# ylsung/vl-merging

Hardware: NVIDIA B200
Metric: gram_cache_samples_per_sec (higher is better)
Workload: dtype tf32

## Files before the change

### include/vlmerge.h

```cpp
#ifndef VLMERGE_H_
#define VLMERGE_H_

#include <stddef.h>
#include <stdint.h>

#ifdef __cplusplus
extern "C" {
#endif

#define VLM_ABI_VERSION 3

typedef enum {
  VLM_OK = 0,
  VLM_ERR_INVALID_ARG = -1,
  VLM_ERR_ALIGNMENT = -2,
  VLM_ERR_UNSUPPORTED = -3,
  VLM_ERR_DRIVER = -4,
  VLM_ERR_NOT_SPD = -5,
  VLM_ERR_INTERNAL = -6
} vlm_status;

typedef enum {
  VLM_F32 = 0, VLM_BF16 = 1, VLM_F16 = 2, VLM_F64 = 3,
  VLM_TF32X2 = 4
} vlm_dtype;

int         vlm_version(void);
const char* vlm_last_error(void);
uint64_t    vlm_launch_count(void);

int vlm_syrk_accum(const void* x, int dtype, int64_t rows, int d, int64_t ldx,
                   float* g, int64_t ldg, void* stream);

int vlm_tf32_split(const float* x, int64_t rows, int d, int64_t ldx, int64_t seg_rows, int64_t seg_stride,
                   float* out, void* stream);

int vlm_syrk_accum_f64(const void* x, int dtype, int64_t rows, int d, int64_t ldx, int64_t seg_rows,
                       int64_t seg_stride, double* g, int64_t ldg, void* stream);

uint64_t vlm_syrk_i8x4_scratch_bytes(int64_t rows, int d);
int vlm_syrk_accum_i8x4(const void* x, int dtype, int64_t rows, int d, int64_t ldx, int64_t seg_rows, int64_t seg_stride,
                        void* scratch, uint64_t scratch_bytes, double* g, int64_t ldg, void* stream);

typedef struct {
  const void* x;
  int64_t     rows;
  int64_t     ldx;
  float*      g;
  int64_t     ldg;
  int32_t     d;
  int32_t     reserved;
  int64_t     seg_rows;
  int64_t     seg_stride;
} vlm_syrk_problem;
int vlm_syrk_accum_batch(const vlm_syrk_problem* probs_host, int n, int dtype, void* stream);

int vlm_syrk_accum_strided(const void* x, int dtype, int64_t rows, int d, int64_t ldx, int64_t seg_rows,
                           int64_t seg_stride, float* g, int64_t ldg, void* stream);

int vlm_syrk_accum_simt(const void* x, int dtype, int64_t rows, int d, int64_t ldx,
                        float* g, int64_t ldg, void* stream);

typedef struct vlm_sym_item {
  const void* full;
  void* packed;
  int32_t d;
  int32_t reserved;
  int64_t ld;
} vlm_sym_item;
int vlm_sym_pack_upper_batch(const vlm_sym_item* items, int n, int dtype, void* stream);
int vlm_sym_unpack_batch(const vlm_sym_item* items, int n, int dtype, void* stream);
int vlm_sym_mirror_batch(const vlm_sym_item* items, int n, int dtype, void* stream);

typedef struct vlm_sym_span {
  uint64_t offset_bytes;
  int32_t d;
  int32_t reserved;
  int64_t ld;
} vlm_sym_span;
int vlm_sym_allreduce_multimem(void* multicast_base, const vlm_sym_span* spans, int n, int dtype, int rank, int world,
                               void* stream);

int vlm_syrk_pair_schedule_host(int64_t rows, int d, int elem_bytes, int nsm, int32_t* segs_out, int cap,
                                int32_t* off_out, int off_cap, int* ncluster_out);

typedef enum { VLM_MERGE_WSUM = 0, VLM_MERGE_SEQ_LERP = 1, VLM_MERGE_MEAN = 2 } vlm_merge_mode;
#define VLM_MERGE_MAX_SRC 4

typedef struct {
  float*       dst;
  const float* src[VLM_MERGE_MAX_SRC];
  float        coef[VLM_MERGE_MAX_SRC];
  uint64_t     n;
  int32_t      n_src;
  int32_t      mode;
} vlm_merge_seg;

typedef struct vlm_merge_plan vlm_merge_plan;
int vlm_merge_plan_create(const vlm_merge_seg* segs_host, int n_seg, vlm_merge_plan** out);
int vlm_merge_plan_run(const vlm_merge_plan* plan, void* stream);
int vlm_merge_plan_destroy(vlm_merge_plan* plan);
uint64_t vlm_merge_plan_bytes(const vlm_merge_plan* plan);

int vlm_copy_batch(void* dst_base, const uint64_t* dst_off_bytes, const void* const* src_host_or_dev,
                   const uint64_t* nbytes, int n, void* stream);

int vlm_gram_scale_accum(const void* g, int g_dtype, int d, int64_t ldg, double alpha,
                         double* out, int64_t ldo, int accumulate, void* stream);
int vlm_regmean_rhs(const float* w, int out_f, int in_f, int64_t ldw,
                    const void* g, int g_dtype, int64_t ldg, double alpha,
                    double* acc, int64_t ldacc, int accumulate, void* stream);
int vlm_regmean_rhs_diff(const float* w, const float* w_base, int out_f, int in_f, int64_t ldw,
                         const void* g, int g_dtype, int64_t ldg, double alpha,
                         double* acc, int64_t ldacc, int accumulate, void* stream);
int vlm_widen_add(const float* src, int rows, int cols, int64_t lds, double* dst, int64_t ldd, void* stream);
int vlm_spd_solve_right(double* s, int in_f, int64_t lds, double* r, int out_f, int64_t ldr,
                        void* stream);
int vlm_spd_solve_right_async(double* s, int in_f, int64_t lds, double* r, int out_f, int64_t ldr,
                              int* info_dev, void* stream);

int vlm_sim_topk_splits(int64_t m, int64_t n);
int vlm_sim_topk(const void* a, int64_t m, int64_t lda, const void* b, int64_t n, int64_t ldb, int d, int dtype,
                 float* out_val, int32_t* out_idx, int splits, void* stream);

int vlm_lu_solve_right(double* s, int in_f, int64_t lds, double* r, int out_f, int64_t ldr, void* stream);

#ifdef __cplusplus
}
#endif
#endif
```

### vl-merging_b200/_lib.py

```python
import ctypes
import itertools
import os
import subprocess
from ctypes import POINTER, c_char_p, c_double, c_float, c_int, c_int32, c_int64, c_uint64, c_void_p

_PKG_DIR = os.path.dirname(os.path.abspath(__file__))
LIB_PATH = os.path.join(_PKG_DIR, "libvlmerge.so")
CSRC_DIR = os.path.join(_PKG_DIR, "csrc")

VLM_F32, VLM_BF16, VLM_F16, VLM_F64, VLM_TF32X2 = 0, 1, 2, 3, 4
MERGE_WSUM, MERGE_SEQ_LERP, MERGE_MEAN = 0, 1, 2
MERGE_MAX_SRC = 4
ERR_NOT_SPD = -5


class MergeSeg(ctypes.Structure):
    _fields_ = [
        ("dst", c_void_p),
        ("src", c_void_p * MERGE_MAX_SRC),
        ("coef", c_float * MERGE_MAX_SRC),
        ("n", c_uint64),
        ("n_src", c_int32),
        ("mode", c_int32),
    ]


class SymItem(ctypes.Structure):
    _fields_ = [("full", c_void_p), ("packed", c_void_p), ("d", c_int32), ("reserved", c_int32), ("ld", c_int64)]


def sym_items(grams, packed=None, offsets=None):
    items = (SymItem * len(grams))()
    if offsets is None:
        offsets = itertools.accumulate((g.shape[0] * (g.shape[0] + 1) // 2 for g in grams), initial=0)
    for it, g, off in zip(items, grams, offsets):
        it.full, it.d, it.ld = g.data_ptr(), g.shape[0], g.stride(0)
        if packed is not None:
            it.packed = packed.data_ptr() + packed.element_size() * off
    return items


class SymSpan(ctypes.Structure):
    _fields_ = [("offset_bytes", ctypes.c_uint64), ("d", c_int32), ("reserved", c_int32), ("ld", c_int64)]


class SyrkProblem(ctypes.Structure):
    _fields_ = [
        ("x", c_void_p),
        ("rows", c_int64),
        ("ldx", c_int64),
        ("g", c_void_p),
        ("ldg", c_int64),
        ("d", c_int32),
        ("reserved", c_int32),
        ("seg_rows", c_int64),
        ("seg_stride", c_int64),
    ]


class VlmError(RuntimeError):
    def __init__(self, code, msg):
        super().__init__(f"libvlmerge error {code}: {msg}")
        self.code = code


SIGNATURES = {
    "vlm_version": (c_int, []),
    "vlm_last_error": (c_char_p, []),
    "vlm_launch_count": (c_uint64, []),
    "vlm_syrk_accum": (c_int, [c_void_p, c_int, c_int64, c_int, c_int64, c_void_p, c_int64, c_void_p]),
    "vlm_tf32_split": (c_int, [c_void_p, c_int64, c_int, c_int64, c_int64, c_int64, c_void_p, c_void_p]),
    "vlm_syrk_accum_f64": (c_int, [c_void_p, c_int, c_int64, c_int, c_int64, c_int64, c_int64, c_void_p, c_int64,
                                   c_void_p]),
    "vlm_syrk_i8x4_scratch_bytes": (c_uint64, [c_int64, c_int]),
    "vlm_syrk_accum_i8x4": (c_int, [c_void_p, c_int, c_int64, c_int, c_int64, c_int64, c_int64, c_void_p, c_uint64,
                                    c_void_p, c_int64, c_void_p]),
    "vlm_syrk_accum_batch": (c_int, [POINTER(SyrkProblem), c_int, c_int, c_void_p]),
    "vlm_syrk_accum_strided": (c_int, [c_void_p, c_int, c_int64, c_int, c_int64, c_int64, c_int64, c_void_p, c_int64,
                                       c_void_p]),
    "vlm_syrk_accum_simt": (c_int, [c_void_p, c_int, c_int64, c_int, c_int64, c_void_p, c_int64, c_void_p]),
    "vlm_sym_pack_upper_batch": (c_int, [POINTER(SymItem), c_int, c_int, c_void_p]),
    "vlm_sym_unpack_batch": (c_int, [POINTER(SymItem), c_int, c_int, c_void_p]),
    "vlm_sym_allreduce_multimem": (c_int, [c_void_p, POINTER(SymSpan), c_int, c_int, c_int, c_int, c_void_p]),
    "vlm_sym_mirror_batch": (c_int, [POINTER(SymItem), c_int, c_int, c_void_p]),
    "vlm_syrk_pair_schedule_host": (c_int, [c_int64, c_int, c_int, c_int, POINTER(c_int32), c_int, POINTER(c_int32),
                                            c_int, POINTER(c_int)]),
    "vlm_merge_plan_create": (c_int, [POINTER(MergeSeg), c_int, POINTER(c_void_p)]),
    "vlm_merge_plan_run": (c_int, [c_void_p, c_void_p]),
    "vlm_merge_plan_destroy": (c_int, [c_void_p]),
    "vlm_merge_plan_bytes": (c_uint64, [c_void_p]),
    "vlm_copy_batch": (c_int, [c_void_p, POINTER(c_uint64), POINTER(c_void_p), POINTER(c_uint64), c_int, c_void_p]),
    "vlm_gram_scale_accum": (c_int, [c_void_p, c_int, c_int, c_int64, c_double, c_void_p, c_int64, c_int, c_void_p]),
    "vlm_regmean_rhs": (c_int, [c_void_p, c_int, c_int, c_int64, c_void_p, c_int, c_int64, c_double, c_void_p,
                                c_int64, c_int, c_void_p]),
    "vlm_regmean_rhs_diff": (c_int, [c_void_p, c_void_p, c_int, c_int, c_int64, c_void_p, c_int, c_int64, c_double,
                                     c_void_p, c_int64, c_int, c_void_p]),
    "vlm_widen_add": (c_int, [c_void_p, c_int, c_int, c_int64, c_void_p, c_int64, c_void_p]),
    "vlm_spd_solve_right": (c_int, [c_void_p, c_int, c_int64, c_void_p, c_int, c_int64, c_void_p]),
    "vlm_sim_topk_splits": (c_int, [c_int64, c_int64]),
    "vlm_sim_topk": (c_int, [c_void_p, c_int64, c_int64, c_void_p, c_int64, c_int64, c_int, c_int, c_void_p, c_void_p, c_int,
                             c_void_p]),
    "vlm_lu_solve_right": (c_int, [c_void_p, c_int, c_int64, c_void_p, c_int, c_int64, c_void_p]),
    "vlm_spd_solve_right_async": (c_int, [c_void_p, c_int, c_int64, c_void_p, c_int, c_int64, c_void_p, c_void_p]),
}

_lib = None


def build(verbose=False):
    res = subprocess.run(["make", "-C", CSRC_DIR, f"-j{min(8, os.cpu_count() or 1)}", "all"], capture_output=True, text=True)
    if verbose or res.returncode != 0:
        print(res.stdout[-4000:])
        print(res.stderr[-4000:])
    if res.returncode != 0:
        raise RuntimeError("building libvlmerge.so failed (see output above)")
    return LIB_PATH


def lib():
    global _lib
    if _lib is None:
        if not os.path.exists(LIB_PATH):
            raise RuntimeError(
                f"{LIB_PATH} not found: build it with `python -c 'import __graft_entry__ as g; g.build()'` "
                "or `make -C vl-merging_b200/csrc`.  There is no CPU fallback for the merge hot path.")
        h = ctypes.CDLL(LIB_PATH)
        for name, (restype, argtypes) in SIGNATURES.items():
            fn = getattr(h, name)
            fn.restype = restype
            fn.argtypes = argtypes
        if h.vlm_version() != 3:
            raise RuntimeError(f"libvlmerge ABI version {h.vlm_version()} != 3: rebuild it (make -C vl-merging_b200/csrc)")
        _lib = h
    return _lib


def check(rc):
    if rc != 0:
        raise VlmError(rc, lib().vlm_last_error().decode(errors="replace"))


def launch_count():
    return int(lib().vlm_launch_count())


def syrk_pair_schedule(rows, d, elem_bytes=4, nsm=148):
    cap = 1 << 16
    segs = (c_int32 * (4 * cap))()
    off = (c_int32 * (nsm + 2))()
    ncl = c_int(0)
    n = lib().vlm_syrk_pair_schedule_host(rows, d, elem_bytes, nsm, segs, cap, off, nsm + 2, ctypes.byref(ncl))
    if n < 0:
        check(n)
    return [tuple(segs[4 * i: 4 * i + 4]) for i in range(n)], list(off[: ncl.value + 1])
```

### vl-merging_b200/model.py

```python
import math

import torch
import torch.nn as nn
import torch.nn.functional as F

MODALITIES = ("v", "l", "vl")


class Mlp(nn.Module):
    def __init__(self, dim, hidden):
        super().__init__()
        self.fc1 = nn.Linear(dim, hidden)
        self.act = nn.GELU()
        self.fc2 = nn.Linear(hidden, dim)

    def forward(self, x):
        return self.fc2(self.act(self.fc1(x)))


class Attention(nn.Module):

    def __init__(self, dim, num_heads, attn_impl="reference"):
        super().__init__()
        self.num_heads = num_heads
        self.scale = (dim // num_heads) ** -0.5
        self.attn_impl = attn_impl
        self.qkv = nn.Linear(dim, dim * 3, bias=False)
        self.q_bias = nn.Parameter(torch.zeros(dim))
        self.v_bias = nn.Parameter(torch.zeros(dim))
        self.proj = nn.Linear(dim, dim)

    def forward(self, x, mask=None, relative_position_bias=None):
        b, n, c = x.shape
        bias = torch.cat((self.q_bias, torch.zeros_like(self.v_bias), self.v_bias))
        qkv = F.linear(x, self.qkv.weight, bias).reshape(b, n, 3, self.num_heads, -1).permute(2, 0, 3, 1, 4)
        if self.attn_impl == "sdpa":
            add = relative_position_bias.unsqueeze(0).to(qkv.dtype) if relative_position_bias is not None else None
            if mask is not None and not bool(mask.all()):
                pad = torch.zeros(b, 1, 1, n, dtype=qkv.dtype, device=x.device).masked_fill(
                    ~mask.bool()[:, None, None, :], float("-inf"))
                add = pad if add is None else add + pad
            x = F.scaled_dot_product_attention(qkv[0], qkv[1], qkv[2], attn_mask=add, scale=self.scale)
            return self.proj(x.transpose(1, 2).reshape(b, n, c))
        q, k, v = qkv[0] * self.scale, qkv[1], qkv[2]
        attn = q.float() @ k.float().transpose(-2, -1)
        if relative_position_bias is not None:
            attn = attn + relative_position_bias.unsqueeze(0)
        if mask is not None:
            attn = attn.masked_fill(~mask.bool()[:, None, None, :], float("-inf"))
        attn = attn.softmax(dim=-1).type_as(x)
        x = (attn @ v).transpose(1, 2).reshape(b, n, c)
        return self.proj(x)


class Block(nn.Module):

    def __init__(self, dim, num_heads, mlp_ratio, experts, attn_impl="reference", joint=False, max_text_len=40):
        super().__init__()
        self.experts = experts
        self.joint = joint
        self.max_text_len = max_text_len
        hidden = int(dim * mlp_ratio)
        ln = lambda: nn.LayerNorm(dim, eps=1e-6)
        if experts is None:
            self.attn, self.norm1 = Attention(dim, num_heads, attn_impl), ln()
            self.mlp, self.norm2 = Mlp(dim, hidden), ln()
        else:
            self.attn = nn.ModuleDict({m: Attention(dim, num_heads, attn_impl) for m in experts})
            self.norm1 = nn.ModuleDict({m: ln() for m in experts})
            self.mlp = nn.ModuleDict({m: Mlp(dim, hidden) for m in experts})
            self.norm2 = nn.ModuleDict({m: ln() for m in experts})
        self.gamma_1 = nn.Parameter(0.1 * torch.ones(dim))
        self.gamma_2 = nn.Parameter(0.1 * torch.ones(dim))

    def forward(self, x, mask, type_id, relative_position_bias):
        if type_id == 2 and not self.joint:
            return self._forward_split(x, mask, relative_position_bias)
        if self.experts is None:
            attn, norm1, mlp, norm2 = self.attn, self.norm1, self.mlp, self.norm2
        else:
            m = MODALITIES[type_id]
            attn, norm1, mlp, norm2 = self.attn[m], self.norm1[m], self.mlp[m], self.norm2[m]
        x = x + self.gamma_1 * attn(norm1(x), mask=mask, relative_position_bias=relative_position_bias)
        x = x + self.gamma_2 * mlp(norm2(x))
        return x

    def _forward_split(self, x, mask, bias):
        L = self.max_text_len
        moe = self.experts is not None
        pick = (lambda mod, m: mod[m]) if moe else (lambda mod, m: mod)
        h = torch.cat([pick(self.norm1, "l")(x[:, :L]), pick(self.norm1, "v")(x[:, L:])], dim=1)
        a_t = pick(self.attn, "l")(h[:, :L], mask=mask[:, :L], relative_position_bias=bias[:, :L, :L])
        a_i = pick(self.attn, "v")(h[:, L:], mask=mask[:, L:], relative_position_bias=bias[:, L:, L:])
        x = x + self.gamma_1 * torch.cat([a_t, a_i], dim=1)
        h = torch.cat([pick(self.norm2, "l")(x[:, :L]), pick(self.norm2, "v")(x[:, L:])], dim=1)
        x = x + self.gamma_2 * torch.cat([pick(self.mlp, "l")(h[:, :L]), pick(self.mlp, "v")(h[:, L:])], dim=1)
        return x


class PatchEmbed(nn.Module):
    def __init__(self, patch_size, dim):
        super().__init__()
        self.proj = nn.Conv2d(3, dim, kernel_size=patch_size, stride=patch_size)

    def forward(self, x):
        return self.proj(x)


class Transformer(nn.Module):
    def __init__(self, cfg, experts_for_layer):
        super().__init__()
        dim = cfg["hidden_size"]
        self.patch_embed = PatchEmbed(cfg["patch_size"], dim)
        self.cls_token = nn.Parameter(torch.zeros(1, 1, dim))
        self.mask_token = nn.Parameter(torch.zeros(1, 1, dim))
        self.blocks = nn.ModuleList(
            [Block(dim, cfg["num_heads"], cfg["mlp_ratio"], experts_for_layer(i), cfg.get("attn_impl", "reference"),
                   joint=i >= cfg["vlffn_start_layer_index"], max_text_len=cfg["max_text_len"])
             for i in range(cfg["num_layers"])])
        self.norm = nn.LayerNorm(dim, eps=1e-6)

    def visual_embed(self, img):
        x = self.patch_embed(img).flatten(2).transpose(1, 2)
        x = torch.cat((self.cls_token.expand(x.shape[0], -1, -1), x), dim=1)
        return x, torch.ones(x.shape[0], x.shape[1], device=x.device)


class TextEmbeddings(nn.Module):

    def __init__(self, vocab_size, dim, max_len):
        super().__init__()
        self.word_embeddings = nn.Embedding(vocab_size, dim, padding_idx=0)
        self.position_embeddings = nn.Embedding(max_len, dim)
        self.token_type_embeddings = nn.Embedding(2, dim)
        self.LayerNorm = nn.LayerNorm(dim, eps=1e-12)

    def forward(self, ids):
        pos = torch.arange(ids.shape[1], device=ids.device)
        x = self.word_embeddings(ids) + self.token_type_embeddings(torch.zeros_like(ids))
        return self.LayerNorm(x + self.position_embeddings(pos)[None])


class _Head(nn.Module):
    def __init__(self, dim, bias):
        super().__init__()
        setattr(self, "fc" if not bias else "dense", nn.Linear(dim, dim, bias=bias))


DEFAULT_CONFIG = dict(
    hidden_size=768, num_heads=12, num_layers=12, mlp_ratio=4, image_size=384, patch_size=16,
    max_text_len=40, max_text_len_of_initckpt=196, vocab_size=30522, vlffn_start_layer_index=10,
    use_moe=True, attn_impl="reference",
)


def vlmo_config(name="base", **overrides):
    cfg = dict(DEFAULT_CONFIG)
    if name == "large":
        cfg.update(hidden_size=1024, num_heads=16, num_layers=24, vlffn_start_layer_index=21)
    elif name == "tiny":
        cfg.update(hidden_size=192, num_heads=3, image_size=224)
    elif name != "base":
        raise ValueError(name)
    cfg.update(overrides)
    return cfg


class VLMo(nn.Module):

    def __init__(self, cfg):
        super().__init__()
        self.cfg = dict(cfg)
        dim, heads, layers = cfg["hidden_size"], cfg["num_heads"], cfg["num_layers"]
        self.num_layers = layers
        self.text_embeddings = TextEmbeddings(cfg["vocab_size"], dim, cfg["max_text_len"])
        self.token_type_embeddings = nn.Embedding(2, dim)
        vl0 = cfg["vlffn_start_layer_index"]
        if cfg["use_moe"]:
            experts = lambda i: ("v", "l") if i < vl0 else ("v", "l", "vl")
        else:
            experts = lambda i: None
        self.transformer = Transformer(cfg, experts)
        self.pooler = _Head(dim, bias=True)
        self.ifm_text_proj = _Head(dim, bias=False)
        self.ifm_image_proj = _Head(dim, bias=False)
        self.logit_scale = nn.Parameter(torch.ones([]) * math.log(1 / 0.07))

        w = cfg["image_size"] // cfg["patch_size"]
        max_text, init_text = cfg["max_text_len"], cfg["max_text_len_of_initckpt"]
        n_img = (2 * w - 1) * (2 * w - 1) + 3
        n_all = n_img + 2 * init_text + 2
        self.relative_position_bias_table = nn.Parameter(torch.zeros(n_all, heads * layers))
        ys, xs = torch.meshgrid(torch.arange(w), torch.arange(w), indexing="ij")
        coords = torch.stack((ys.flatten(), xs.flatten()))
        rel = (coords[:, :, None] - coords[:, None, :]).permute(1, 2, 0)
        idx = torch.zeros(w * w + 1, w * w + 1, dtype=torch.long)
        idx[1:, 1:] = (rel[..., 0] + w - 1) * (2 * w - 1) + rel[..., 1] + w - 1
        idx[0, :] = n_img - 3
        idx[:, 0] = n_img - 2
        idx[0, 0] = n_img - 1
        self.register_buffer("relative_position_index", idx)
        pos = torch.arange(max_text - 1)
        tidx = torch.zeros(max_text, max_text, dtype=torch.long)
        tidx[1:, 1:] = (pos[None, :] - pos[:, None]) - (2 - init_text) + n_img + 2
        tidx[0, :] = n_all - 3
        tidx[:, 0] = n_all - 2
        tidx[0, 0] = n_all - 1
        self.register_buffer("text_relative_position_index", tidx)
        t2i = torch.full((max_text, w * w + 1), float(n_img))
        i2t = torch.full((w * w + 1, max_text), float(n_img + 1))
        self.register_buffer("text_imag_relative_position_index",
                             torch.cat((torch.cat((tidx.float(), t2i), 1), torch.cat((i2t, idx.float()), 1)), 0))

    def _rel_pos_bias(self, index):
        bias = F.embedding(index, self.relative_position_bias_table).permute(2, 0, 1).contiguous()
        return torch.chunk(bias, self.num_layers, dim=0)

    def infer_text_ft(self, batch):
        ids, masks = batch["text_ids"], batch["text_masks"]
        x = self.text_embeddings(ids) + self.token_type_embeddings(torch.zeros_like(masks))
        biases = self._rel_pos_bias(self.text_relative_position_index)
        for i, blk in enumerate(self.transformer.blocks):
            x = blk(x, masks, 1, biases[i])
        feats = self.transformer.norm(x)
        cls = self.ifm_text_proj.fc(feats[:, 0])
        return {"text_feats": feats, "cls_feats": cls / cls.norm(dim=-1, keepdim=True), "raw_cls_feats": x[:, 0]}

    def infer_image_ft(self, batch, image_token_type_idx=1):
        img = batch["image"][0] if isinstance(batch["image"], (list, tuple)) else batch["image"]
        x, masks = self.transformer.visual_embed(img)
        masks = masks.long()
        x = x + self.token_type_embeddings(torch.full_like(masks, image_token_type_idx))
        biases = self._rel_pos_bias(self.relative_position_index)
        for i, blk in enumerate(self.transformer.blocks):
            x = blk(x, masks, 0, biases[i])
        feats = self.transformer.norm(x)
        cls = self.ifm_image_proj.fc(feats[:, 0])
        return {"image_feats": feats, "cls_feats": cls / cls.norm(dim=-1, keepdim=True), "raw_cls_feats": x[:, 0]}

    def infer(self, batch, image_token_type_idx=1):
        img = batch["image"][0] if isinstance(batch["image"], (list, tuple)) else batch["image"]
        ids, text_masks = batch["text_ids"], batch["text_masks"]
        text = self.text_embeddings(ids)
        image, image_masks = self.transformer.visual_embed(img)
        image_masks = image_masks.type_as(text_masks)
        text = text + self.token_type_embeddings(torch.zeros_like(text_masks))
        image = image + self.token_type_embeddings(torch.full_like(image_masks, image_token_type_idx))
        x = torch.cat([text, image], dim=1)
        masks = torch.cat([text_masks, image_masks], dim=1)
        biases = self._rel_pos_bias(self.text_imag_relative_position_index.long())
        for i, blk in enumerate(self.transformer.blocks):
            x = blk(x, masks, 2, biases[i])
        x = self.transformer.norm(x)
        n_text = text.shape[1]
        return {"text_feats": x[:, :n_text], "image_feats": x[:, n_text:],
                "cls_feats": torch.tanh(self.pooler.dense(x[:, 0])), "raw_cls_feats": x[:, 0]}

    def forward(self, batch):
        img = self.infer_image_ft(batch)["cls_feats"]
        txt = self.infer_text_ft(batch)["cls_feats"]
        return self.logit_scale.exp() * img @ txt.t()



def _hash_uniform(numel, seed, device="cpu"):
    i = torch.arange(numel, dtype=torch.int64, device=device)
    x = ((i + 1) * 0x9E3779B1 + (seed % (1 << 24)) * 0x85EBCA77 + 0x165667B1) % (1 << 32)
    x = (x ^ (x >> 15)) * 0x2C1B3C6D % (1 << 32)
    x = (x ^ (x >> 12)) * 0x297A2D39 % (1 << 32)
    x = x ^ (x >> 15)
    return ((x % (1 << 24)).to(torch.float32) + 0.5) / float(1 << 24) - 0.5


@torch.no_grad()
def init_synthetic_(model, seed=1):
    import zlib

    for name, p in model.named_parameters():
        u = _hash_uniform(p.numel(), seed * 1000003 + zlib.crc32(name.encode()) % 999983, device=p.device).reshape(p.shape)
        if "norm" in name.lower() and name.endswith("weight"):
            p.copy_(1.0 + 0.2 * u)
        elif "gamma_" in name:
            p.copy_(0.1 + 0.05 * u)
        elif name == "logit_scale":
            p.fill_(math.log(1 / 0.07))
        elif name.endswith("bias") or "cls_token" in name or "mask_token" in name:
            p.copy_(0.1 * u)
        elif name == "relative_position_bias_table":
            p.copy_(0.5 * u)
        else:
            p.copy_(0.07 * u)
    return model


def synthetic_batch(batch_size, cfg, seed=0, device="cpu", dtype=torch.float32, pad=False):
    n = batch_size * 3 * cfg["image_size"] ** 2
    image = (2.0 * _hash_uniform(n, 7919 + seed)).reshape(batch_size, 3, cfg["image_size"], cfg["image_size"])
    t = cfg["max_text_len"]
    ids = ((_hash_uniform(batch_size * t, 104729 + seed) + 0.5) * (cfg["vocab_size"] - 1000)).long() + 999
    ids = ids.reshape(batch_size, t)
    ids[:, 0] = 101
    masks = torch.ones(batch_size, t, dtype=torch.long)
    if pad:
        lens = 8 + ((_hash_uniform(batch_size, 31 + seed) + 0.5) * (t - 8)).long()
        masks = (torch.arange(t)[None, :] < lens[:, None]).long()
        ids = ids * masks
    return {
        "image": [image.to(device=device, dtype=dtype)],
        "text_ids": ids.to(device),
        "text_masks": masks.to(device),
        "text_labels": torch.full((batch_size, t), -100, dtype=torch.long, device=device),
    }
```

Before: 1217.

## Add fused tcgen05 flash-attention forward kernel with split-TF32 for sdpa path

Adds a native Blackwell attention forward kernel. It splits QKV into TF32 high and low planes, loads tiles with TMA, runs QK^T and PV on tcgen05 UMMA with results held in tensor memory, and does an online softmax with bias and mask staged in shared memory. The model's sdpa branch routes fp32 head_dim-64 inference attention through this kernel, replacing the PyTorch SDPA call with its materialized additive mask and bias. In exchange it needs a scratch buffer twice the size of qkv and an extra split launch per call, and it adds substantial hand-written descriptor logic.

```diff
diff --git a/include/vlmerge.h b/include/vlmerge.h
--- a/include/vlmerge.h
+++ b/include/vlmerge.h
@@ -125,6 +125,11 @@
 
 int vlm_lu_solve_right(double* s, int in_f, int64_t lds, double* r, int out_f, int64_t ldr, void* stream);
 
+int vlm_attention_fwd(const float* qkv, int batch, int n, int heads, int head_dim, float scale,
+                      const float* bias, int64_t bias_head_stride, int64_t bias_row_stride,
+                      const int64_t* key_mask, int64_t mask_batch_stride, float* scratch, float* out,
+                      void* stream);
+
 #ifdef __cplusplus
 }
 #endif
diff --git a/vl-merging_b200/_lib.py b/vl-merging_b200/_lib.py
--- a/vl-merging_b200/_lib.py
+++ b/vl-merging_b200/_lib.py
@@ -102,6 +102,8 @@
                              c_void_p]),
     "vlm_lu_solve_right": (c_int, [c_void_p, c_int, c_int64, c_void_p, c_int, c_int64, c_void_p]),
     "vlm_spd_solve_right_async": (c_int, [c_void_p, c_int, c_int64, c_void_p, c_int, c_int64, c_void_p, c_void_p]),
+    "vlm_attention_fwd": (c_int, [c_void_p, c_int, c_int, c_int, c_int, c_float, c_void_p, c_int64, c_int64, c_void_p,
+                                  c_int64, c_void_p, c_void_p, c_void_p]),
 }
 
 _lib = None
diff --git a/vl-merging_b200/csrc/attention.cu b/vl-merging_b200/csrc/attention.cu
--- /dev/null
+++ b/vl-merging_b200/csrc/attention.cu
@@ -0,0 +1,378 @@
+#include <algorithm>
+
+#include "common.cuh"
+#include "syrk.h"
+
+namespace vlm {
+namespace {
+
+constexpr int aBM = 128, aBN = 64, aD = 64;
+constexpr int aThreads = 128;
+constexpr int aQBytes = 2 * 2 * aBM * 128;
+constexpr int aKVBytes = 2 * 2 * aBN * 128;
+constexpr int aBiasPitch = aBN + 1;
+constexpr int aBiasBytes = aBM * aBiasPitch * 4;
+constexpr int aSmemBytes = aQBytes + 4 * aKVBytes + aBiasBytes + aBN * 4 + 128 + 1024;
+constexpr uint32_t aTmemCols = 512;
+constexpr float kLog2e = 1.4426950408889634f;
+
+__device__ __forceinline__ void tma_load_3d(const CUtensorMap* tm, uint64_t* bar, void* smem_dst, int c0, int c1, int c2) {
+  asm volatile(
+      "cp.async.bulk.tensor.3d.shared::cluster.global.mbarrier::complete_tx::bytes [%0], [%1, {%3, %4, %5}], [%2];"
+      ::"r"(smem_u32(smem_dst)), "l"(reinterpret_cast<uint64_t>(tm)), "r"(smem_u32(bar)), "r"(c0), "r"(c1), "r"(c2)
+      : "memory");
+}
+__device__ __forceinline__ void tmem_st_32x32b_x32(uint32_t taddr, const uint32_t (&v)[32]) {
+  asm volatile(
+      "tcgen05.st.sync.aligned.32x32b.x32.b32 [%0], "
+      "{%1, %2, %3, %4, %5, %6, %7, %8, %9, %10, %11, %12, %13, %14, %15, %16, "
+      "%17, %18, %19, %20, %21, %22, %23, %24, %25, %26, %27, %28, %29, %30, %31, %32};"
+      ::"r"(taddr), "r"(v[0]), "r"(v[1]), "r"(v[2]), "r"(v[3]), "r"(v[4]), "r"(v[5]), "r"(v[6]), "r"(v[7]), "r"(v[8]),
+        "r"(v[9]), "r"(v[10]), "r"(v[11]), "r"(v[12]), "r"(v[13]), "r"(v[14]), "r"(v[15]), "r"(v[16]), "r"(v[17]),
+        "r"(v[18]), "r"(v[19]), "r"(v[20]), "r"(v[21]), "r"(v[22]), "r"(v[23]), "r"(v[24]), "r"(v[25]), "r"(v[26]),
+        "r"(v[27]), "r"(v[28]), "r"(v[29]), "r"(v[30]), "r"(v[31])
+      : "memory");
+}
+__device__ __forceinline__ void cp_async_4(void* smem_dst, const void* src, uint32_t src_bytes) {
+  asm volatile("cp.async.ca.shared.global [%0], [%1], 4, %2;" ::"r"(smem_u32(smem_dst)), "l"(src), "r"(src_bytes) : "memory");
+}
+__device__ __forceinline__ void cp_async_wait_all() { asm volatile("cp.async.wait_all;" ::: "memory"); }
+__device__ __forceinline__ void tmem_st_wait() { asm volatile("tcgen05.wait::st.sync.aligned;" ::: "memory"); }
+__device__ __forceinline__ void umma_ss(uint32_t d_tmem, uint64_t adesc, uint64_t bdesc, uint32_t idesc, uint32_t acc) {
+  asm volatile(
+      "{\n\t.reg .pred p;\n\tsetp.ne.b32 p, %4, 0;\n\t"
+      "tcgen05.mma.cta_group::1.kind::tf32 [%0], %1, %2, %3, p;\n\t}\n" ::"r"(d_tmem),
+      "l"(adesc), "l"(bdesc), "r"(idesc), "r"(acc)
+      : "memory");
+}
+__device__ __forceinline__ void umma_ts(uint32_t d_tmem, uint32_t a_tmem, uint64_t bdesc, uint32_t idesc, uint32_t acc) {
+  asm volatile(
+      "{\n\t.reg .pred p;\n\tsetp.ne.b32 p, %4, 0;\n\t"
+      "tcgen05.mma.cta_group::1.kind::tf32 [%0], [%1], %2, %3, p;\n\t}\n" ::"r"(d_tmem),
+      "r"(a_tmem), "l"(bdesc), "r"(idesc), "r"(acc)
+      : "memory");
+}
+__device__ __forceinline__ float tf32_rna(float v) {
+  uint32_t r;
+  asm("cvt.rna.tf32.f32 %0, %1;" : "=r"(r) : "f"(v));
+  return __uint_as_float(r);
+}
+
+constexpr uint32_t kIdescS = (1u << 4) | (2u << 7) | (2u << 10) | ((uint32_t)(aBN >> 3) << 17) | ((uint32_t)(aBM >> 4) << 24);
+constexpr uint32_t kIdescPV = kIdescS | (1u << 16);
+constexpr uint32_t kKmajHi = (uint32_t)(1024 >> 4) | (1u << 14) | (2u << 29);
+constexpr uint32_t kKmajLo = (uint32_t)(16 >> 4) << 16;
+constexpr uint32_t kMNHi = (uint32_t)(512 >> 4) | (1u << 14) | (1u << 29);
+constexpr uint32_t kMNLo = (uint32_t)((aBN * 128) >> 4) << 16;
+__device__ __forceinline__ uint64_t sdesc(uint32_t hi, uint32_t lo, uint32_t addr) {
+  return ((uint64_t)hi << 32) | (lo | ((addr & 0x3FFFFu) >> 4));
+}
+
+__global__ void __launch_bounds__(aThreads, 1)
+attention_fwd_kernel(const __grid_constant__ CUtensorMap tm_qk, const __grid_constant__ CUtensorMap tm_v, int B, int N,
+                     int H, float scale, const float* __restrict__ bias, int64_t bias_hs, int64_t bias_rs,
+                     const int64_t* __restrict__ key_mask, int64_t mask_bs, float* __restrict__ out) {
+  extern __shared__ uint8_t smem_raw[];
+  uint8_t* smem = reinterpret_cast<uint8_t*>((reinterpret_cast<uintptr_t>(smem_raw) + 1023) & ~uintptr_t(1023));
+  uint8_t* sq = smem;
+  uint8_t* sk = sq + aQBytes;
+  uint8_t* sv = sk + 2 * aKVBytes;
+  float* sbias = reinterpret_cast<float*>(sv + 2 * aKVBytes);
+  float* smadd = sbias + aBM * aBiasPitch;
+  uint64_t* bars = reinterpret_cast<uint64_t*>(smadd + aBN);
+  uint64_t* qbar = bars;
+  uint64_t* kfull = bars + 1;
+  uint64_t* vfull = bars + 3;
+  uint64_t* sbar = bars + 5;
+  uint64_t* pvbar = bars + 7;
+  uint32_t* tmem_slot = reinterpret_cast<uint32_t*>(bars + 9);
+
+  const int tid = threadIdx.x, warp = tid >> 5, lane = tid & 31;
+  const int nqt = (N + aBM - 1) / aBM;
+  const int q0 = (int)(blockIdx.x % nqt) * aBM;
+  const int bh = (int)(blockIdx.x / nqt);
+  const int b = bh / H, h = bh - b * H;
+  const int nt = (N + aBN - 1) / aBN;
+  const int col_q = h * aD, col_k = (H + h) * aD, col_v = (2 * H + h) * aD;
+
+  if (tid == 0) {
+    tma_prefetch_desc(&tm_qk);
+    tma_prefetch_desc(&tm_v);
+    mbar_init(qbar, 1);
+    for (int i = 0; i < 2; ++i) {
+      mbar_init(&kfull[i], 1);
+      mbar_init(&vfull[i], 1);
+      mbar_init(&sbar[i], 1);
+      mbar_init(&pvbar[i], 1);
+    }
+    fence_barrier_init();
+  }
+  __syncwarp();
+  if (warp == 0) {
+    tmem_alloc(tmem_slot, aTmemCols);
+    tmem_relinquish();
+  }
+  tc_fence_before();
+  __syncthreads();
+  tc_fence_after();
+  const uint32_t tmem = *tmem_slot;
+  const uint32_t t_s = tmem, t_ph = tmem + 128, t_pl = tmem + 256, t_pv = tmem + 384;
+
+  auto load_k = [&](int j) {
+    uint8_t* dst = sk + (j & 1) * aKVBytes;
+    mbar_arrive_expect_tx(&kfull[j & 1], aKVBytes);
+    for (int p = 0; p < 2; ++p)
+      for (int c = 0; c < 2; ++c) tma_load_3d(&tm_qk, &kfull[j & 1], dst + (2 * p + c) * 8192, col_k + 32 * c, j * aBN, p * B + b);
+  };
+  auto load_v = [&](int j) {
+    uint8_t* dst = sv + (j & 1) * aKVBytes;
+    mbar_arrive_expect_tx(&vfull[j & 1], aKVBytes);
+    for (int p = 0; p < 2; ++p)
+      for (int c = 0; c < 2; ++c) tma_load_3d(&tm_v, &vfull[j & 1], dst + (2 * p + c) * 8192, col_v + 32 * c, j * aBN, p * B + b);
+  };
+  auto issue_s = [&](int j) {
+    const uint32_t qa = smem_u32(sq), ka = smem_u32(sk + (j & 1) * aKVBytes);
+    const uint32_t d = t_s + (j & 1) * aBN;
+#pragma unroll
+    for (int pass = 0; pass < 2; ++pass)
+#pragma unroll
+      for (int kk = 0; kk < aD / 8; ++kk) {
+        const uint32_t qo = (kk >> 2) * (aBM * 128) + (kk & 3) * 32, ko = (kk >> 2) * (aBN * 128) + (kk & 3) * 32;
+        const uint64_t qh = sdesc(kKmajHi, kKmajLo, qa + qo), ql = sdesc(kKmajHi, kKmajLo, qa + aQBytes / 2 + qo);
+        const uint64_t kh = sdesc(kKmajHi, kKmajLo, ka + ko), kl = sdesc(kKmajHi, kKmajLo, ka + aKVBytes / 2 + ko);
+        if (pass == 0) {
+          umma_ss(d, qh, kl, kIdescS, kk > 0 ? 1u : 0u);
+          umma_ss(d, ql, kh, kIdescS, 1u);
+        } else {
+          umma_ss(d, qh, kh, kIdescS, 1u);
+        }
+      }
+    tc_commit(&sbar[j & 1]);
+  };
+  auto issue_pv = [&](int j) {
+    const uint32_t va = smem_u32(sv + (j & 1) * aKVBytes);
+    const uint32_t d = t_pv + (j & 1) * aD, ph = t_ph + (j & 1) * aBN, pl = t_pl + (j & 1) * aBN;
+#pragma unroll
+    for (int pass = 0; pass < 2; ++pass)
+#pragma unroll
+      for (int kk = 0; kk < aBN / 8; ++kk) {
+        const uint64_t vh = sdesc(kMNHi, kMNLo, va + kk * 1024), vl = sdesc(kMNHi, kMNLo, va + aKVBytes / 2 + kk * 1024);
+        if (pass == 0) {
+          umma_ts(d, ph + kk * 8, vl, kIdescPV, kk > 0 ? 1u : 0u);
+          umma_ts(d, pl + kk * 8, vh, kIdescPV, 1u);
+        } else {
+          umma_ts(d, ph + kk * 8, vh, kIdescPV, 1u);
+        }
+      }
+    tc_commit(&pvbar[j & 1]);
+  };
+
+  if (tid == 0) {
+    mbar_arrive_expect_tx(qbar, aQBytes);
+    for (int p = 0; p < 2; ++p)
+      for (int c = 0; c < 2; ++c)
+        for (int r = 0; r < 2; ++r)
+          tma_load_3d(&tm_qk, qbar, sq + p * (aQBytes / 2) + c * (aBM * 128) + r * (aBN * 128), col_q + 32 * c,
+                      q0 + r * aBN, p * B + b);
+    load_k(0);
+    load_v(0);
+    if (nt > 1) {
+      load_k(1);
+      load_v(1);
+    }
+    mbar_wait(qbar, 0);
+    mbar_wait(&kfull[0], 0);
+    tc_fence_after();
+    issue_s(0);
+    if (nt > 1) {
+      mbar_wait(&kfull[1], 0);
+      tc_fence_after();
+      issue_s(1);
+    }
+  }
+  __syncwarp();
+
+  const int row = tid;
+  const int q = q0 + row;
+  const uint32_t lane_off = (uint32_t)(warp * 32) << 16;
+  const float sl2 = scale * kLog2e;
+  const float* bias_bh = bias ? bias + (int64_t)h * bias_hs : nullptr;
+  float m = -INFINITY, l = 0.f, alpha_prev = 0.f;
+  float o[aD];
+#pragma unroll
+  for (int i = 0; i < aD; ++i) o[i] = 0.f;
+
+  auto fold_pv = [&](int j, float alpha) {
+    mbar_wait(&pvbar[j & 1], (j >> 1) & 1);
+    tc_fence_after();
+    uint32_t v[32];
+#pragma unroll
+    for (int hf = 0; hf < 2; ++hf) {
+      tmem_ld_32x32b_x32(t_pv + lane_off + (j & 1) * aD + 32 * hf, v);
+      tmem_ld_wait();
+#pragma unroll
+      for (int i = 0; i < 32; ++i) o[32 * hf + i] = fmaf(o[32 * hf + i], alpha, __uint_as_float(v[i]));
+    }
+  };
+
+  auto stage_bias_mask = [&](int j) {
+    const int k0 = j * aBN;
+    if (bias_bh) {
+      for (int r = warp; r < aBM; r += aThreads / 32) {
+        const int qr = q0 + r;
+#pragma unroll
+        for (int c = lane; c < aBN; c += 32) {
+          const int k = k0 + c;
+          const bool in = qr < N && k < N;
+          cp_async_4(&sbias[r * aBiasPitch + c], in ? bias_bh + (int64_t)qr * bias_rs + k : bias_bh, in ? 4u : 0u);
+        }
+      }
+    }
+    if (tid < aBN) {
+      const int k = k0 + tid;
+      smadd[tid] = (k < N && (key_mask == nullptr || key_mask[(int64_t)b * mask_bs + k] != 0)) ? 0.f : -INFINITY;
+    }
+  };
+  stage_bias_mask(0);
+
+  for (int j = 0; j < nt; ++j) {
+    const int buf = j & 1;
+    const uint32_t par = (j >> 1) & 1;
+    cp_async_wait_all();
+    tc_fence_before();
+    __syncthreads();
+
+    mbar_wait(&sbar[buf], par);
+    tc_fence_after();
+    if (tid == 0 && j + 2 < nt) load_k(j + 2);
+    __syncwarp();
+
+    float s[aBN];
+    {
+      uint32_t v[32];
+#pragma unroll
+      for (int hf = 0; hf < 2; ++hf) {
+        tmem_ld_32x32b_x32(t_s + lane_off + buf * aBN + 32 * hf, v);
+        tmem_ld_wait();
+#pragma unroll
+        for (int i = 0; i < 32; ++i) s[32 * hf + i] = __uint_as_float(v[i]);
+      }
+    }
+    float tmax = -INFINITY;
+#pragma unroll
+    for (int c = 0; c < aBN; ++c) {
+      const float add = bias_bh ? fmaf(sbias[row * aBiasPitch + c], kLog2e, smadd[c]) : smadd[c];
+      s[c] = fmaf(s[c], sl2, add);
+      tmax = fmaxf(tmax, s[c]);
+    }
+    const float m_new = fmaxf(m, tmax);
+    const float m_use = m_new == -INFINITY ? 0.f : m_new;
+    const float alpha = exp2f(m - m_use);
+    float rsum = 0.f;
+#pragma unroll
+    for (int hf = 0; hf < 2; ++hf) {
+      uint32_t phi[32], plo[32];
+#pragma unroll
+      for (int i = 0; i < 32; ++i) {
+        const float p = exp2f(s[32 * hf + i] - m_use);
+        rsum += p;
+        const float ph = tf32_rna(p);
+        phi[i] = __float_as_uint(ph);
+        plo[i] = __float_as_uint(tf32_rna(p - ph));
+      }
+      tmem_st_32x32b_x32(t_ph + lane_off + buf * aBN + 32 * hf, phi);
+      tmem_st_32x32b_x32(t_pl + lane_off + buf * aBN + 32 * hf, plo);
+    }
+    l = fmaf(l, alpha, rsum);
+    m = m_new;
+    tmem_st_wait();
+    tc_fence_before();
+    __syncthreads();
+
+    if (tid == 0) {
+      tc_fence_after();
+      mbar_wait(&vfull[buf], par);
+      tc_fence_after();
+      issue_pv(j);
+      if (j + 2 < nt) {
+        mbar_wait(&kfull[buf], par ^ 1);
+        tc_fence_after();
+        issue_s(j + 2);
+      }
+    }
+    __syncwarp();
+    if (j + 1 < nt) stage_bias_mask(j + 1);
+    if (j >= 1) {
+      fold_pv(j - 1, alpha_prev);
+      if (tid == 0 && j + 1 < nt) load_v(j + 1);
+      __syncwarp();
+    }
+    alpha_prev = alpha;
+  }
+  fold_pv(nt - 1, alpha_prev);
+
+  if (q < N) {
+    const float inv = 1.f / l;
+    float4* dst = reinterpret_cast<float4*>(out + ((int64_t)b * N + q) * (int64_t)(H * aD) + h * aD);
+#pragma unroll
+    for (int i = 0; i < aD / 4; ++i)
+      dst[i] = make_float4(o[4 * i] * inv, o[4 * i + 1] * inv, o[4 * i + 2] * inv, o[4 * i + 3] * inv);
+  }
+  tc_fence_before();
+  __syncthreads();
+  if (warp == 0) tmem_dealloc(tmem, aTmemCols);
+}
+
+int encode_qkv_map(const float* planes, int B, int N, int H, CUtensorMapSwizzle swz, CUtensorMap* tm) {
+  EncodeTiledFn encode = nullptr;
+  if (int rc = tensor_map_encoder(&encode)) return rc;
+  const uint64_t c = 3ull * H * aD;
+  cuuint64_t gdim[3] = {(cuuint64_t)c, (cuuint64_t)N, (cuuint64_t)(2 * B)};
+  cuuint64_t gstr[2] = {(cuuint64_t)(c * 4), (cuuint64_t)(c * 4 * N)};
+  cuuint32_t box[3] = {32, (cuuint32_t)aBN, 1};
+  cuuint32_t estr[3] = {1, 1, 1};
+  CUresult r = encode(tm, CU_TENSOR_MAP_DATA_TYPE_FLOAT32, 3, const_cast<float*>(planes), gdim, gstr, box, estr,
+                      CU_TENSOR_MAP_INTERLEAVE_NONE, swz, CU_TENSOR_MAP_L2_PROMOTION_L2_256B, CU_TENSOR_MAP_FLOAT_OOB_FILL_NONE);
+  VLM_REQUIRE(r == CUDA_SUCCESS, VLM_ERR_DRIVER, "cuTensorMapEncodeTiled(qkv planes) failed: CUresult %d", (int)r);
+  return 0;
+}
+
+}
+}
+
+using namespace vlm;
+
+extern "C" int vlm_attention_fwd(const float* qkv, int batch, int n, int heads, int head_dim, float scale,
+                                 const float* bias, int64_t bias_head_stride, int64_t bias_row_stride,
+                                 const int64_t* key_mask, int64_t mask_batch_stride, float* scratch, float* out,
+                                 void* stream) {
+  VLM_REQUIRE(qkv && scratch && out, VLM_ERR_INVALID_ARG, "vlm_attention_fwd: qkv, scratch and out must not be NULL");
+  VLM_REQUIRE(head_dim == aD, VLM_ERR_UNSUPPORTED, "vlm_attention_fwd: head_dim must be 64 (got %d)", head_dim);
+  VLM_REQUIRE(batch > 0 && heads > 0 && n > 0 && (int64_t)batch * heads * ((n + aBM - 1) / aBM) < ((int64_t)1 << 31),
+              VLM_ERR_INVALID_ARG, "vlm_attention_fwd: bad shape (batch=%d n=%d heads=%d)", batch, n, heads);
+  VLM_REQUIRE((int64_t)batch * n * 3 * heads * aD < ((int64_t)1 << 40), VLM_ERR_INVALID_ARG, "vlm_attention_fwd: qkv too large");
+  VLM_REQUIRE(bias == nullptr || (bias_head_stride >= 0 && bias_row_stride >= n), VLM_ERR_INVALID_ARG,
+              "vlm_attention_fwd: bias strides must be non-negative with bias_row_stride >= n");
+  VLM_REQUIRE(key_mask == nullptr || mask_batch_stride >= 0, VLM_ERR_INVALID_ARG,
+              "vlm_attention_fwd: mask_batch_stride must be non-negative");
+  VLM_REQUIRE((reinterpret_cast<uintptr_t>(qkv) & 15) == 0 && (reinterpret_cast<uintptr_t>(scratch) & 15) == 0 &&
+                  (reinterpret_cast<uintptr_t>(out) & 15) == 0,
+              VLM_ERR_ALIGNMENT, "vlm_attention_fwd: qkv, scratch and out must be 16-byte aligned");
+  VLM_REQUIRE((reinterpret_cast<uintptr_t>(bias) & 3) == 0 && (reinterpret_cast<uintptr_t>(key_mask) & 7) == 0,
+              VLM_ERR_ALIGNMENT, "vlm_attention_fwd: bias must be 4-byte and key_mask 8-byte aligned");
+  if (int rc = require_sm100()) return rc;
+  cudaStream_t st = static_cast<cudaStream_t>(stream);
+  const int64_t rows = (int64_t)batch * n;
+  const int c = 3 * heads * aD;
+  if (int rc = tf32_split_launch(qkv, rows, c, c, 0, 0, scratch, st)) return rc;
+  CUtensorMap tm_qk, tm_v;
+  if (int rc = encode_qkv_map(scratch, batch, n, heads, CU_TENSOR_MAP_SWIZZLE_128B, &tm_qk)) return rc;
+  if (int rc = encode_qkv_map(scratch, batch, n, heads, CU_TENSOR_MAP_SWIZZLE_128B_ATOM_32B, &tm_v)) return rc;
+  VLM_CUDA(cudaFuncSetAttribute(attention_fwd_kernel, cudaFuncAttributeMaxDynamicSharedMemorySize, aSmemBytes));
+  const unsigned grid = (unsigned)((int64_t)batch * heads * ((n + aBM - 1) / aBM));
+  attention_fwd_kernel<<<grid, aThreads, aSmemBytes, st>>>(tm_qk, tm_v, batch, n, heads, scale, bias, bias_head_stride,
+                                                            bias_row_stride, key_mask, mask_batch_stride, out);
+  VLM_CUDA(cudaGetLastError());
+  count_launch();
+  return 0;
+}
diff --git a/vl-merging_b200/model.py b/vl-merging_b200/model.py
--- a/vl-merging_b200/model.py
+++ b/vl-merging_b200/model.py
@@ -4,6 +4,8 @@
 import torch.nn as nn
 import torch.nn.functional as F
 
+from . import _lib
+
 MODALITIES = ("v", "l", "vl")
 
 
@@ -16,6 +18,32 @@
 
     def forward(self, x):
         return self.fc2(self.act(self.fc1(x)))
+
+
+def native_attention_applies(qkv, head_dim, bias=None):
+    if not (qkv.is_cuda and qkv.dtype == torch.float32 and head_dim == 64
+            and torch.cuda.get_device_capability(qkv.device)[0] == 10):
+        return False
+    return not (torch.is_grad_enabled() and (qkv.requires_grad or (bias is not None and bias.requires_grad)))
+
+
+def native_attention(qkv, num_heads, scale, bias=None, mask=None):
+    b, n, _ = qkv.shape
+    qkv = qkv.contiguous()
+    scratch = torch.empty(2 * qkv.numel(), dtype=torch.float32, device=qkv.device)
+    out = torch.empty(b, n, qkv.shape[-1] // 3, dtype=torch.float32, device=qkv.device)
+    if bias is not None and (bias.dtype != torch.float32 or bias.stride(-1) != 1):
+        bias = bias.float().contiguous()
+    if mask is not None and (mask.dtype != torch.int64 or mask.stride(-1) != 1):
+        mask = mask.to(torch.int64).contiguous()
+    stream = torch.cuda.current_stream(qkv.device).cuda_stream
+    _lib.check(_lib.lib().vlm_attention_fwd(
+        qkv.data_ptr(), b, n, num_heads, 64, scale,
+        bias.data_ptr() if bias is not None else None, bias.stride(0) if bias is not None else 0,
+        bias.stride(1) if bias is not None else 0,
+        mask.data_ptr() if mask is not None else None, mask.stride(0) if mask is not None else 0,
+        scratch.data_ptr(), out.data_ptr(), stream))
+    return out
 
 
 class Attention(nn.Module):
@@ -33,7 +61,10 @@
     def forward(self, x, mask=None, relative_position_bias=None):
         b, n, c = x.shape
         bias = torch.cat((self.q_bias, torch.zeros_like(self.v_bias), self.v_bias))
-        qkv = F.linear(x, self.qkv.weight, bias).reshape(b, n, 3, self.num_heads, -1).permute(2, 0, 3, 1, 4)
+        qkv = F.linear(x, self.qkv.weight, bias)
+        if self.attn_impl == "sdpa" and native_attention_applies(qkv, c // self.num_heads, relative_position_bias):
+            return self.proj(native_attention(qkv, self.num_heads, self.scale, relative_position_bias, mask))
+        qkv = qkv.reshape(b, n, 3, self.num_heads, -1).permute(2, 0, 3, 1, 4)
         if self.attn_impl == "sdpa":
             add = relative_position_bias.unsqueeze(0).to(qkv.dtype) if relative_position_bias is not None else None
             if mask is not None and not bool(mask.all()):
```

Result: faster. 1361 (median of 6 runs) (+11.9%).
